# qiaozhijian/VCR-Net

Measured on NVIDIA B200. Metric: pairs/sec @1024 pts, higher is better.
Workload: dtype f16x3-split+f32acc (fp32-equivalent)

## Files before the change

### include/vcr_b200.h

```cpp
#ifndef VCR_B200_H
#define VCR_B200_H

#include <stddef.h>
#include <stdint.h>

#ifdef __cplusplus
extern "C" {
#endif

#ifndef __CUDA_RUNTIME_H__
typedef struct CUstream_st* cudaStream_t;
#endif

long long vcr_launch_count(void);
int vcr_abi_version(void);

size_t vcr_knn_workspace_bytes(int B, int N);
int vcr_knn_topk(const float* x, int B, int D, int N, int k, int token_major, int32_t* idx32,
                 int64_t* idx64, void* workspace, size_t workspace_bytes, cudaStream_t stream);

int vcr_set_knn3_direct(int on);
int vcr_set_knn_tc_tpq(int on);

size_t vcr_knn_tc_workspace_bytes(int B, int N);
int vcr_knn_topk_tc(const float* x, const void* xop, int ld, long long plane_stride, int B, int D, int N, int k,
                    int32_t* idx32, int64_t* idx64, void* workspace, size_t workspace_bytes, cudaStream_t stream);

int vcr_graph_feature(const float* xt, int B, int D, int N, int k, const int* idx, float* out,
                      cudaStream_t stream);

int vcr_fps(const float* xyz, int B, int N, int npoint, int32_t* idx32, int64_t* idx64, cudaStream_t stream);

int vcr_gemm_f32(const float* A, int lda, long long sAo, long long sAi,
                 const float* B, int ldb, long long sBo, long long sBi, int b_layout,
                 float* C, int ldc, long long sCo, long long sCi,
                 const float* bias, const float* residual, int ldr, long long sRo, long long sRi,
                 int M, int N, int K, int nb_outer, int nb_inner,
                 float alpha, int act, float slope, cudaStream_t stream);

int vcr_gemm_tc(const void* A, int lda, long long a_rows_total, int a_cols_total, long long a_plane,
                long long a_row_o, long long a_row_i, int a_col_o, int a_col_i,
                const void* B, int ldb, long long b_rows_total, int b_cols_total, long long b_plane,
                long long b_row_o, long long b_row_i, int b_col_o, int b_col_i,
                int M, int N, int K, int nb_outer, int nb_inner, int mode,
                float alpha, const float* bias, int act, float slope,
                float* C, int ldc, long long c_so, long long c_si,
                const float* R, int ldr, long long r_so, long long r_si,
                void* H, int ldh, long long h_plane, long long h_so, long long h_si, int h_split,
                void* HT, int ldt, long long t_plane, long long t_so, long long t_si,
                int out_planes, cudaStream_t stream);
int vcr_flash_attn_tc(const void* Q, int ldq, long long q_plane, const void* K, int ldk, long long k_plane,
                      const void* VT, int ldv, long long v_plane, int B, int H, int Nq, int Nk, int dk,
                      int mode, float scale, const uint8_t* keep, void* O, int ldo, long long o_plane,
                      float* lse, cudaStream_t stream);
int vcr_set_flash_warps(int nwq);
int vcr_set_gemm_pair(int on);
int vcr_gemm_quad_clusters(void);
int vcr_to_operand(const float* x, int ld, long long rows, int cols, void* out, int ldo, long long plane_stride,
                   int planes, int bf16, cudaStream_t stream);

int vcr_conv3_act(const float* xyz, const float* w, const float* bias, int B, int N, int Cout, float slope,
                  float* out, int ldo, cudaStream_t stream);
int vcr_edgeconv_dg(const float* PQ, int ldpq, const int* idx, int k, int N, long long total_pts,
                    const float* W2, const float* b2, float slope, float* x1, int ld1, float* x2, int ld2,
                    cudaStream_t stream);
int vcr_edgeconv_dg_tc(const float* PQ, int ldpq, const int* idx, int k, int N, long long total_pts,
                       const float* W2, const float* b2, float slope, int mode, float* x1, int ld1,
                       float* x2, int ld2, void* op1, void* op2, int ldop, long long op_plane, float* z,
                       cudaStream_t stream);
int vcr_gather_max(const float* P, int ldp, const float* Q, int ldq, const int* idx, int k, int N,
                   long long total_pts, int C, float slope, float* out, int ldo, void* op, int ldop,
                   long long op_plane, cudaStream_t stream);
int vcr_lpd_point_mlp(const float* xyz, const float* w1, const float* b1, const float* w2, const float* b2, int B, int N,
                      float slope, float* h1, float* h2, void* op, int ldop, long long op_plane, cudaStream_t stream);

int vcr_layernorm(const float* x, int ldx, const float* a, const float* b, float eps, long long M, int D,
                  const float* residual, int ldr, float* out, int ldo, cudaStream_t stream);
int vcr_layernorm_head(const float* x, int ldx, const float* a, const float* b, float eps, long long M, int D,
                       const float* residual, int ldr, float* out, int ldo, void* op, int ldop,
                       long long plane_stride, float* sq, cudaStream_t stream);
int vcr_softmax_rows(float* S, int ld, long long rows, int n, const uint8_t* keep, long long rows_per_batch,
                     cudaStream_t stream);
size_t vcr_colsum_workspace_bytes(int B, int n);
int vcr_colsum(const float* P, int ld, int B, long long rows_per_batch, int n, float* out, void* workspace,
               size_t workspace_bytes, cudaStream_t stream);
int vcr_layernorm_operand(const float* x, int ldx, const float* a, const float* b, float eps, long long M, int D,
                          void* out, int ldo, long long plane_stride, int planes, int bf16, cudaStream_t stream);
int vcr_row_lse(const float* S, int ld, long long rows, int n, const uint8_t* keep, long long rows_per_batch,
                float* rmax, float* rsum, cudaStream_t stream);
int vcr_softmax_operand(const float* S, int ld, long long rows, int n, const uint8_t* keep,
                        long long rows_per_batch, void* out, int ldo, long long plane_stride, int planes,
                        int bf16, cudaStream_t stream);
size_t vcr_attn_colsum_workspace_bytes(int B, int H, int Nq, int Nk);
int vcr_attn_colsum_tc(const void* Q, int ldq, long long q_plane, const void* K, int ldk, long long k_plane,
                       int B, int H, int Nq, int Nk, int dk, float scale, float* out, void* workspace,
                       size_t workspace_bytes, cudaStream_t stream);
size_t vcr_softmax_colsum_workspace_bytes(int B, long long rows_per_batch, int ld, int n);
int vcr_softmax_colsum(const float* S, int ld, int B, long long rows_per_batch, int n, float* out,
                       void* workspace, size_t workspace_bytes, cudaStream_t stream);
int vcr_colsum_softmax(const float* S, int ld, int B, long long rows_per_batch, int n, const float* rmax,
                       const float* rsum, float* out, void* workspace, size_t workspace_bytes, cudaStream_t stream);
int vcr_rowsum(const float* P, int ld, long long rows, int n, float* out, cudaStream_t stream);
int vcr_topk_select(const float* vals, int B, int n, int K, int* idx_out, uint8_t* mask_out, cudaStream_t stream);

int vcr_sqnorm_rows(const float* X, int ld, long long rows, int D, float* out, cudaStream_t stream);
int vcr_softcorr_rows(float* dot, int ld, int B, int Ns, int Nt, const float* xx, const float* yy,
                      const float* tgt, int mode, float* corr, int* best_idx, float* best_val, cudaStream_t stream);
int vcr_negdist(float* dot, int ld, int B, int Ns, int Nt, const float* xx, const float* yy, cudaStream_t stream);
int vcr_softcorr_tc(const void* S, int lds, long long s_plane, const void* T, int ldt, long long t_plane,
                    const float* xx, const float* yy, const float* tgt, int B, int Ns, int Nt, int D,
                    float* corr, cudaStream_t stream);
int vcr_softcorr_best_tc(const void* S, int lds, long long s_plane, const void* T, int ldt, long long t_plane,
                         const float* xx, const float* yy, int B, int Ns, int Nt, int D,
                         int* best_idx, float* best_val, cudaStream_t stream);
size_t vcr_select_stats_tc_workspace_bytes(int B, int Ns, int Nt);
int vcr_select_stats_tc(const void* S, int lds, long long s_plane, const void* T, int ldt, long long t_plane,
                        const float* xx, const float* yy, int B, int Ns, int Nt, int D, float* row_stat, float* col_stat,
                        void* workspace, size_t workspace_bytes, cudaStream_t stream);
size_t vcr_rowsum_colsoftmax_workspace_bytes(int B, int Nt);
int vcr_rowsum_colsoftmax(const float* pd, int ld, int B, int Ns, int Nt, float* out, void* workspace,
                          size_t workspace_bytes, cudaStream_t stream);
size_t vcr_select_stats_workspace_bytes(int B, int Ns, int Nt);
int vcr_select_stats(const float* dot, int ld, int B, int Ns, int Nt, const float* xx, const float* yy,
                     float* row_stat, float* col_stat, void* workspace, size_t workspace_bytes, cudaStream_t stream);
int vcr_gather_operand_rows(const void* in, int ld_in, long long plane_in, int B, int Nin, const int* idx, int K,
                            int C, void* out, int ld_out, long long plane_out, const float* sq_in, float* sq_out,
                            cudaStream_t stream);
int vcr_gather_rows(const float* in, int ld_in, int B, int Nin, const int* idx, int K, int C, float* out,
                    int ld_out, cudaStream_t stream);
int vcr_gather_cols(const float* in, int B, int C, int Nin, const int* idx, int K, float* out, cudaStream_t stream);
int vcr_copair_gather(const float* src, const float* tgt, int B, int Ns, int Nt, const int* keep,
                      const int* best_idx, int K, float* src_out, float* corr_out, cudaStream_t stream);

int vcr_svd_head(const float* src, const float* corr, int B, int M, float* R_ab, float* t_ab,
                 float* R_ba, float* t_ba, float* H_out, cudaStream_t stream);
int vcr_rigid_apply(const float* pc, const float* R, const float* t, int B, int N, float* out, cudaStream_t stream);
int vcr_pose_compose(const float* R_i, const float* t_i, float* R_f, float* t_f, int B, cudaStream_t stream);
int vcr_pose_inverse(const float* R, const float* t, float* R_inv, float* t_inv, int B, cudaStream_t stream);
int vcr_host_svd3(const double* H, double* U, double* S, double* V);

int vcr_transpose(const float* in, float* out, int nb, int R, int C, int ld_in, int ld_out,
                  long long stride_in, long long stride_out, cudaStream_t stream);
int vcr_add(const float* a, const float* b, float* out, long long n, cudaStream_t stream);

int vcr_make_pairs(const float* base, int P, int Nb, const int* idx_src, const int* idx_tgt, const double* pose,
                   int N, double* src64, double* tgt64, float* src, float* tgt, cudaStream_t stream);
int vcr_crop_nearest(const double* pc64, int P, int N, int keep, float* out, cudaStream_t stream);
size_t vcr_crop_nearest_workspace_bytes(int P, int N);
int vcr_crop_nearest_sort(const double* pc64, int P, int N, int keep, float* out, void* workspace, size_t workspace_bytes,
                          cudaStream_t stream);
int vcr_eval_metrics(const float* src, const float* tgt, int N, const float* srcK, const float* corrK, int M,
                     const float* R_gt, const float* t_gt, const float* R_ab, const float* t_ab,
                     const float* R_ba, const float* t_ba, int B, double* acc, cudaStream_t stream);

size_t vcr_icp_state_bytes(void);
int vcr_icp_nearest(const float* src, const float* dst, int B, int Ns, int Nt, float* corr, int* nn_idx,
                    double* err_sum, cudaStream_t stream);
int vcr_icp_advance(float* src, const float* R, const float* t, int B, int Ns, const double* err_sum,
                    float tolerance, void* state, cudaStream_t stream);

int vcr_edge_max(const float* E, int k, long long total_pts, int C, float* out, int ldo, cudaStream_t stream);

int vcr_wgrad_f32(const float* G, int ldg, const float* X, int ldx, long long M, int N, int K, float* dW,
                  int lddw, float* db, cudaStream_t stream);
int vcr_act_bwd(const float* gy, int ldg, const float* y, int ldy, long long rows, int cols, float slope,
                const int* scale_bits, float* gz, int ldz, cudaStream_t stream);
int vcr_absmax_bits(const float* x, long long n, int* bits, cudaStream_t stream);
int vcr_pow2_inverse(const int* bits, float* out, cudaStream_t stream);
int vcr_gather_max_bwd(const float* P, int ldp, const float* Q, int ldq, const int* idx, int k, int N,
                       long long total_pts, int C, float slope, const float* gout, int ldgo, float* gP,
                       int ldgp, float* gQ, int ldgq, cudaStream_t stream);
int vcr_edge_gather_act(const float* PQ, int ldpq, const int* idx, int k, int N, long long total_pts, int C,
                        float slope, float* E, cudaStream_t stream);
int vcr_edge_max_bwd(float* Z, const float* gx, int ldgx, int k, long long total_pts, int C, float slope,
                     cudaStream_t stream);
int vcr_edge_bwd_scatter(const float* E, const float* gE, const float* gx1, int ldgx, const int* idx, int k,
                         int N, long long total_pts, int C, float slope, float* gPQ, int ldg,
                         cudaStream_t stream);

#ifdef __cplusplus
}
#endif
#endif
```

### vcr_net_b200/csrc/knn.cu

```cuda
#include <atomic>
#include "tc_common.cuh"

namespace {

constexpr int TQ = 32;
constexpr int TC = 512;
constexpr int NT = 256;
constexpr int RPL = TC / 32;

template <bool TOKEN_MAJOR>
__global__ void knn_sqnorm_kernel(const float* __restrict__ x, int D, int N, float* __restrict__ xx) {
    const int b = blockIdx.y;
    const int i = blockIdx.x * blockDim.x + threadIdx.x;
    if (i >= N) return;
    const float* xb = x + (size_t)b * D * N;
    float acc = 0.f;
    for (int d = 0; d < D; ++d) {
        const float v = TOKEN_MAJOR ? xb[(size_t)i * D + d] : xb[(size_t)d * N + i];
        acc = fmaf(v, v, acc);
    }
    xx[(size_t)b * N + i] = acc;
}

__device__ __forceinline__ uint32_t okey(float v) {
    const uint32_t b = __float_as_uint(v + 0.f);
    return b ^ (uint32_t)(((int32_t)b >> 31) | 0x80000000);
}
__device__ __forceinline__ float okey_inv(uint32_t k) {
    return __uint_as_float((k & 0x80000000u) ? (k ^ 0x80000000u) : ~k);
}
struct Key { uint32_t hi, lo; };
__device__ __forceinline__ Key key_xchg(Key v, int j, bool take_max) {
    Key o;
    o.hi = __shfl_xor_sync(0xffffffffu, v.hi, j);
    o.lo = __shfl_xor_sync(0xffffffffu, v.lo, j);
    const bool gt = v.hi > o.hi || (v.hi == o.hi && v.lo > o.lo);
    return gt == take_max ? v : o;
}
__device__ __forceinline__ Key key_max(Key a, Key b) {
    return (a.hi > b.hi || (a.hi == b.hi && a.lo > b.lo)) ? a : b;
}

template <int W>
__device__ __forceinline__ void sort32_desc(Key (&v)[W], int lane) {
#pragma unroll
    for (int ks = 2; ks <= 32; ks <<= 1) {
#pragma unroll
        for (int j = ks >> 1; j > 0; j >>= 1) {
            const bool take_max = ((lane & j) == 0) == ((lane & ks) == 0);
#pragma unroll
            for (int w = 0; w < W; ++w) v[w] = key_xchg(v[w], j, take_max);
        }
    }
}
template <int W>
__device__ __forceinline__ void sort32_desc_f(float (&v)[W], int lane) {
#pragma unroll
    for (int ks = 2; ks <= 32; ks <<= 1) {
#pragma unroll
        for (int j = ks >> 1; j > 0; j >>= 1) {
            const bool take_max = ((lane & j) == 0) == ((lane & ks) == 0);
#pragma unroll
            for (int w = 0; w < W; ++w) {
                const float o = __shfl_xor_sync(0xffffffffu, v[w], j);
                v[w] = take_max ? fmaxf(v[w], o) : fminf(v[w], o);
            }
        }
    }
}
template <int W>
__device__ __forceinline__ void merge32_desc(Key (&run)[W], const Key (&add)[W], int lane) {
#pragma unroll
    for (int w = 0; w < W; ++w) {
        Key o;
        o.hi = __shfl_sync(0xffffffffu, add[w].hi, 31 - lane);
        o.lo = __shfl_sync(0xffffffffu, add[w].lo, 31 - lane);
        run[w] = key_max(run[w], o);
    }
#pragma unroll
    for (int j = 16; j > 0; j >>= 1) {
        const bool take_max = (lane & j) == 0;
#pragma unroll
        for (int w = 0; w < W; ++w) run[w] = key_xchg(run[w], j, take_max);
    }
}

template <int W, int TCN, int LDD, int CAP>
__device__ __forceinline__ bool filter_merge_t(const float* drows, const float (&tau)[W], Key (&run)[W], uint2* buf,
                                               int j0, int lane) {
    constexpr int RP = TCN / 32;
    const uint32_t lt = (1u << lane) - 1u;
    int cnt[W], off[W];
    int base = 0;
    __syncwarp();
#pragma unroll
    for (int w = 0; w < W; ++w) {
        const float* dr = drows + w * LDD + lane;
        float v[RP];
#pragma unroll
        for (int r = 0; r < RP; ++r) v[r] = dr[r * 32];
        off[w] = base;
        int n = base;
#pragma unroll
        for (int r = 0; r < RP; ++r) {
            const bool p = v[r] >= tau[w];
            const uint32_t bal = __ballot_sync(0xffffffffu, p);
            const int pos = n + __popc(bal & lt);
            if (p && pos < CAP) buf[pos] = make_uint2(~(uint32_t)(j0 + r * 32 + lane), okey(v[r]));
            n += __popc(bal);
        }
        cnt[w] = n - base;
        base = n;
    }
    __syncwarp();
    if (base > CAP) return false;
    int rounds = 0;
#pragma unroll
    for (int w = 0; w < W; ++w) rounds = max(rounds, (cnt[w] + 31) >> 5);
    for (int r = 0; r < rounds; ++r) {
        Key e[W];
#pragma unroll
        for (int w = 0; w < W; ++w) {
            const int p = r * 32 + lane;
            const uint2 t = p < cnt[w] ? buf[off[w] + p] : make_uint2(0u, 0u);
            e[w].lo = t.x; e[w].hi = t.y;
        }
        sort32_desc<W>(e, lane);
        merge32_desc<W>(run, e, lane);
    }
    return true;
}
template <int W>
__device__ __forceinline__ bool filter_merge(const float* drows, const float (&tau)[W], Key (&run)[W], uint2* buf,
                                             int j0, int lane) {
    return filter_merge_t<W, TC, TC, TC>(drows, tau, run, buf, j0, lane);
}

__device__ __forceinline__ void select_chunk(const float* dist, uint2* surv, Key (&run)[TQ / (NT / 32)], int j0, int kk,
                                             int warp, int lane, bool first) {
    constexpr int QWn = TQ / (NT / 32);
    uint2* buf = surv + (size_t)warp * TC;
    const float* drows = dist + (size_t)(warp * QWn) * TC;
    float tau[QWn];
    if (first) {
        float m[QWn];
#pragma unroll
        for (int w = 0; w < QWn; ++w) {
            const float* dr = drows + w * TC + lane;
            float mm = dr[0];
#pragma unroll
            for (int r = 1; r < RPL; ++r) mm = fmaxf(mm, dr[r * 32]);
            m[w] = mm;
        }
        sort32_desc_f<QWn>(m, lane);
#pragma unroll
        for (int w = 0; w < QWn; ++w) tau[w] = __shfl_sync(0xffffffffu, m[w], kk);
    } else {
#pragma unroll
        for (int w = 0; w < QWn; ++w) tau[w] = okey_inv(__shfl_sync(0xffffffffu, run[w].hi, kk));
    }
    if (!filter_merge<QWn>(drows, tau, run, buf, j0, lane)) {
#pragma unroll
        for (int w = 0; w < QWn; ++w) {
            float t1[1] = {tau[w]};
            Key r1[1] = {run[w]};
            filter_merge<1>(drows + w * TC, t1, r1, buf, j0, lane);
            run[w] = r1[0];
        }
    }
}

__device__ __forceinline__ void cp_async16(float* dst, const float* src, bool valid) {
    const uint32_t d = (uint32_t)__cvta_generic_to_shared(dst);
    const int sz = valid ? 16 : 0;
    asm volatile("cp.async.ca.shared.global [%0], [%1], 16, %2;\n" ::"r"(d), "l"(src), "r"(sz) : "memory");
}
__device__ __forceinline__ void cp_async_wait_all() { asm volatile("cp.async.wait_all;\n" ::: "memory"); }
__device__ __forceinline__ void cp_async_commit() { asm volatile("cp.async.commit_group;\n" ::: "memory"); }
template <int NPEND>
__device__ __forceinline__ void cp_async_wait_group() { asm volatile("cp.async.wait_group %0;\n" ::"n"(NPEND) : "memory"); }

template <int DCH, int DCP>
__device__ __forceinline__ void issue_slab(const float* __restrict__ xb, int D, int N, int j0, int q0, int d0,
                                           float* Cb, float* Qb, int tid) {
    constexpr int PPR = DCH / 4;
    constexpr int RPP = 256 / PPR;
    const int part = tid % PPR, r0 = tid / PPR;
    const bool dok = d0 + 4 * part < D;
    const float* src = xb + (size_t)(j0 + r0) * D + d0 + 4 * part;
    float* dst = Cb + r0 * DCP + 4 * part;
#pragma unroll
    for (int n = 0; n < 512 / RPP; ++n) {
        const bool ok = dok && j0 + r0 + n * RPP < N;
        cp_async16(dst + n * RPP * DCP, ok ? src + (size_t)n * RPP * D : xb, ok);
    }
    if (r0 < 32) {
        const bool ok = dok && q0 + r0 < N;
        cp_async16(Qb + r0 * DCP + 4 * part, ok ? xb + (size_t)(q0 + r0) * D + d0 + 4 * part : xb, ok);
    }
    cp_async_commit();
}

constexpr int QW = TQ / (NT / 32);
constexpr size_t SURV_BYTES = (size_t)(NT / 32) * TC * sizeof(uint2);

template <int DCH>
struct Smem {
    static constexpr int DCP = DCH == 4 ? 12 : DCH + 4;
    static constexpr size_t stage_bytes = (size_t)(TC + TQ) * DCP * sizeof(float);
    static constexpr size_t region0 = stage_bytes > SURV_BYTES ? stage_bytes : SURV_BYTES;
    static constexpr size_t total = region0 + (size_t)TC * sizeof(float) + (size_t)TQ * TC * sizeof(float);
};

template <int DCH, bool TOKEN_MAJOR>
__global__ void __launch_bounds__(NT, 2)
knn_select_kernel(const float* __restrict__ x, const float* __restrict__ xx, int D, int N, int k,
                  int32_t* __restrict__ idx32, int64_t* __restrict__ idx64, const int* __restrict__ redo) {
    if (redo != nullptr && redo[blockIdx.y * gridDim.x + blockIdx.x] == 0) return;
    using S = Smem<DCH>;
    constexpr int DCP = S::DCP;
    extern __shared__ __align__(16) unsigned char smem_raw[];
    float* Cs = reinterpret_cast<float*>(smem_raw);
    float* Qs = Cs + TC * DCP;
    uint2* surv = reinterpret_cast<uint2*>(smem_raw);
    float* xxc = reinterpret_cast<float*>(smem_raw + S::region0);
    float* dist = xxc + TC;

    const int tid = threadIdx.x, lane = tid & 31, warp = tid >> 5;
    const int qg = warp & 3, cg = warp >> 2;
    const int b = blockIdx.y, q0 = blockIdx.x * TQ;
    const float* xb = x + (size_t)b * D * N;
    const float* xxb = xx + (size_t)b * N;
    const bool vec = TOKEN_MAJOR && (D % 4 == 0) && ((reinterpret_cast<uintptr_t>(x) & 15) == 0);

    Key run[QW];
#pragma unroll
    for (int w = 0; w < QW; ++w) run[w].hi = run[w].lo = 0u;

    for (int j0 = 0; j0 < N; j0 += TC) {
        float acc[8][8];
#pragma unroll
        for (int qi = 0; qi < 8; ++qi)
#pragma unroll
            for (int ci = 0; ci < 8; ++ci) acc[qi][ci] = 0.f;

        const int nslab = (D + DCH - 1) / DCH;
        __syncthreads();
        if (vec) issue_slab<DCH, DCP>(xb, D, N, j0, q0, 0, Cs, Qs, tid);
        for (int c = tid; c < TC; c += NT) xxc[c] = (j0 + c < N) ? xxb[j0 + c] : 0.f;
        for (int si = 0; si < nslab; ++si) {
            const int d0 = si * DCH;
            const float* Cb = (vec && (si & 1)) ? dist : Cs;
            const float* Qb = Cb + TC * DCP;
            if (vec) {
                if (si + 1 < nslab) {
                    float* Cn = (si & 1) ? Cs : dist;
                    issue_slab<DCH, DCP>(xb, D, N, j0, q0, d0 + DCH, Cn, Cn + TC * DCP, tid);
                    cp_async_wait_group<1>();
                } else {
                    cp_async_wait_group<0>();
                }
            } else {
                for (int e = tid; e < (TC + TQ) * DCH; e += NT) {
                    int row, d;
                    if (TOKEN_MAJOR) { row = e / DCH; d = e - row * DCH; }
                    else if (e < TC * DCH) { d = e / TC; row = e - d * TC; }
                    else { const int e2 = e - TC * DCH; d = e2 / TQ; row = TC + e2 - d * TQ; }
                    const int g = row < TC ? j0 + row : q0 + (row - TC);
                    float v = 0.f;
                    if (g < N && d0 + d < D)
                        v = TOKEN_MAJOR ? xb[(size_t)g * D + d0 + d] : xb[(size_t)(d0 + d) * N + g];
                    Cs[row * DCP + d] = v;
                }
            }
            __syncthreads();

            const float* qrow = Qb + (qg * 8) * DCP;
            const float* crow = Cb + (cg * 256 + lane) * DCP;
            if (j0 + cg * 256 < N) {
#pragma unroll 1
            for (int d4 = 0; d4 < DCH / 4; ++d4) {
#pragma unroll
                for (int h = 0; h < 2; ++h) {
                    float4 cv[4];
#pragma unroll
                    for (int ci = 0; ci < 4; ++ci)
                        cv[ci] = *reinterpret_cast<const float4*>(crow + ((h * 4 + ci) * 32) * DCP + d4 * 4);
#pragma unroll
                    for (int qi = 0; qi < 8; ++qi) {
                        const float4 qv = *reinterpret_cast<const float4*>(qrow + qi * DCP + d4 * 4);
#pragma unroll
                        for (int ci = 0; ci < 4; ++ci) acc[qi][h * 4 + ci] = fmaf(qv.x, cv[ci].x, acc[qi][h * 4 + ci]);
#pragma unroll
                        for (int ci = 0; ci < 4; ++ci) acc[qi][h * 4 + ci] = fmaf(qv.y, cv[ci].y, acc[qi][h * 4 + ci]);
#pragma unroll
                        for (int ci = 0; ci < 4; ++ci) acc[qi][h * 4 + ci] = fmaf(qv.z, cv[ci].z, acc[qi][h * 4 + ci]);
#pragma unroll
                        for (int ci = 0; ci < 4; ++ci) acc[qi][h * 4 + ci] = fmaf(qv.w, cv[ci].w, acc[qi][h * 4 + ci]);
                    }
                }
            }
            }
            __syncthreads();
        }

        float xxq[8];
#pragma unroll
        for (int qi = 0; qi < 8; ++qi) {
            const int q = q0 + qg * 8 + qi;
            xxq[qi] = q < N ? xxb[q] : 0.f;
        }
#pragma unroll
        for (int ci = 0; ci < 8; ++ci) {
            const int c = cg * 256 + ci * 32 + lane;
            const float nxc = -xxc[c];
            const bool cvalid = j0 + c < N;
#pragma unroll
            for (int qi = 0; qi < 8; ++qi) {
                const float pd = __fsub_rn(__fsub_rn(nxc, -2.f * acc[qi][ci]), xxq[qi]);
                dist[(qg * 8 + qi) * TC + c] = cvalid ? pd : -INFINITY;
            }
        }
        __syncthreads();

        select_chunk(dist, surv, run, j0, k, warp, lane, j0 == 0);
    }

#pragma unroll
    for (int w = 0; w < QW; ++w) {
        const int q = q0 + warp * QW + w;
        if (q < N && lane >= 1 && lane <= k) {
            const int j = (int)(~run[w].lo);
            const size_t o = ((size_t)b * N + q) * k + lane - 1;
            if (idx32) idx32[o] = j;
            if (idx64) idx64[o] = (int64_t)j;
        }
    }
}

template <int DCH, bool TM>
int launch_knn(const float* x, const float* xx, int B, int D, int N, int k, int32_t* i32, int64_t* i64,
               cudaStream_t st, const int* redo = nullptr) {
    auto kern = knn_select_kernel<DCH, TM>;
    const size_t smem = Smem<DCH>::total;
    if (cudaFuncSetAttribute(kern, cudaFuncAttributeMaxDynamicSharedMemorySize, (int)smem) != cudaSuccess) return VCR_ERR_LAUNCH;
    dim3 grid(vcr_cdiv(N, TQ), B);
    kern<<<grid, NT, smem, st>>>(x, xx, D, N, k, i32, i64, redo);
    VCR_CHECK_LAUNCH();
    return VCR_OK;
}

template <int W, class F>
__device__ __forceinline__ bool filter_merge_fn(F&& get, const float (&tau)[W], Key (&run)[W], uint2* buf, int j0, int lane) {
    constexpr int RP = TC / 32;
    const uint32_t lt = (1u << lane) - 1u;
    int cnt[W], off[W];
    int base = 0;
    __syncwarp();
#pragma unroll
    for (int w = 0; w < W; ++w) {
        off[w] = base;
        int n = base;
#pragma unroll
        for (int r = 0; r < RP; ++r) {
            const float v = get(w, r);
            const bool p = v >= tau[w];
            const uint32_t bal = __ballot_sync(0xffffffffu, p);
            const int pos = n + __popc(bal & lt);
            if (p && pos < TC) buf[pos] = make_uint2(~(uint32_t)(j0 + r * 32 + lane), okey(v));
            n += __popc(bal);
        }
        cnt[w] = n - base;
        base = n;
    }
    __syncwarp();
    if (base > TC) return false;
    int rounds = 0;
#pragma unroll
    for (int w = 0; w < W; ++w) rounds = max(rounds, (cnt[w] + 31) >> 5);
    for (int r = 0; r < rounds; ++r) {
        Key e[W];
#pragma unroll
        for (int w = 0; w < W; ++w) {
            const int p = r * 32 + lane;
            const uint2 t = p < cnt[w] ? buf[off[w] + p] : make_uint2(0u, 0u);
            e[w].lo = t.x; e[w].hi = t.y;
        }
        sort32_desc<W>(e, lane);
        merge32_desc<W>(run, e, lane);
    }
    return true;
}

constexpr int QW3 = 2;
constexpr int TQ3 = QW3 * (NT / 32);
template <bool TOKEN_MAJOR>
__global__ void __launch_bounds__(NT, 4)
knn3_kernel(const float* __restrict__ x, const float* __restrict__ xx, int N, int k,
            int32_t* __restrict__ idx32, int64_t* __restrict__ idx64) {
    __shared__ float cs[4][TC];
    __shared__ uint2 surv[NT / 32][TC];
    const int tid = threadIdx.x, lane = tid & 31, warp = tid >> 5;
    const int b = blockIdx.y, q0 = blockIdx.x * TQ3;
    const float* xb = x + (size_t)b * 3 * N;
    const float* xxb = xx + (size_t)b * N;

    float qx[QW3], qy[QW3], qz[QW3], xxq[QW3];
#pragma unroll
    for (int w = 0; w < QW3; ++w) {
        const int q = min(q0 + warp * QW3 + w, N - 1);
        qx[w] = TOKEN_MAJOR ? xb[(size_t)q * 3 + 0] : xb[q];
        qy[w] = TOKEN_MAJOR ? xb[(size_t)q * 3 + 1] : xb[(size_t)N + q];
        qz[w] = TOKEN_MAJOR ? xb[(size_t)q * 3 + 2] : xb[2 * (size_t)N + q];
        xxq[w] = xxb[q];
    }
    Key run[QW3];
#pragma unroll
    for (int w = 0; w < QW3; ++w) run[w].hi = run[w].lo = 0u;
    uint2* buf = surv[warp];

    for (int j0 = 0; j0 < N; j0 += TC) {
        __syncthreads();
        for (int c = tid; c < TC; c += NT) {
            const int g = j0 + c;
            const bool ok = g < N;
            cs[0][c] = ok ? (TOKEN_MAJOR ? xb[(size_t)g * 3 + 0] : xb[g]) : 0.f;
            cs[1][c] = ok ? (TOKEN_MAJOR ? xb[(size_t)g * 3 + 1] : xb[(size_t)N + g]) : 0.f;
            cs[2][c] = ok ? (TOKEN_MAJOR ? xb[(size_t)g * 3 + 2] : xb[2 * (size_t)N + g]) : 0.f;
            cs[3][c] = ok ? xxb[g] : 0.f;
        }
        __syncthreads();
        auto pd = [&](int w, int r) -> float {
            const int c = r * 32 + lane;
            const float acc = fmaf(qz[w], cs[2][c], fmaf(qy[w], cs[1][c], fmaf(qx[w], cs[0][c], 0.f)));
            const float v = __fsub_rn(__fsub_rn(-cs[3][c], -2.f * acc), xxq[w]);
            return j0 + c < N ? v : -INFINITY;
        };
        float tau[QW3];
        if (j0 == 0) {
            float m[QW3];
#pragma unroll
            for (int w = 0; w < QW3; ++w) {
                float mm = pd(w, 0);
#pragma unroll
                for (int r = 1; r < RPL; ++r) mm = fmaxf(mm, pd(w, r));
                m[w] = mm;
            }
            sort32_desc_f<QW3>(m, lane);
#pragma unroll
            for (int w = 0; w < QW3; ++w) tau[w] = __shfl_sync(0xffffffffu, m[w], k);
        } else {
#pragma unroll
            for (int w = 0; w < QW3; ++w) tau[w] = okey_inv(__shfl_sync(0xffffffffu, run[w].hi, k));
        }
        if (!filter_merge_fn<QW3>(pd, tau, run, buf, j0, lane)) {
#pragma unroll
            for (int w = 0; w < QW3; ++w) {
                float t1[1] = {tau[w]};
                Key r1[1] = {run[w]};
                filter_merge_fn<1>([&](int, int r) { return pd(w, r); }, t1, r1, buf, j0, lane);
                run[w] = r1[0];
            }
        }
    }
#pragma unroll
    for (int w = 0; w < QW3; ++w) {
        const int q = q0 + warp * QW3 + w;
        if (q < N && lane >= 1 && lane <= k) {
            const int j = (int)(~run[w].lo);
            const size_t o = ((size_t)b * N + q) * k + lane - 1;
            if (idx32) idx32[o] = j;
            if (idx64) idx64[o] = (int64_t)j;
        }
    }
}

constexpr int T2M = 128;
constexpr int T2TILES = TC / T2M;
constexpr int T2NT = NT + 32;
constexpr int T2CTILE = T2M * 128;
constexpr int T2QTILE = TQ * 128;

struct KnnTcParams {
    const float* x;
    const float* xx;
    const uint32_t* xxmax;
    int* redo;
    int* nflag;
    int D, N, k, ksel, KB;
    int32_t* idx32;
    int64_t* idx64;
};

__host__ __device__ constexpr size_t knn_tc_stage_bytes(int KB) {
    return (size_t)KB * 2 * T2CTILE > SURV_BYTES ? (size_t)KB * 2 * T2CTILE : SURV_BYTES;
}
__host__ __device__ constexpr size_t knn_tc_smem_bytes(int KB) {
    return (size_t)KB * 2 * T2QTILE + knn_tc_stage_bytes(KB) + (size_t)TQ * TC * 4 + TQ * 4 + 64 + 1024;
}

__global__ void knn_sqnorm_max_kernel(const float* __restrict__ x, int D, int N, float* __restrict__ xx,
                                      uint32_t* __restrict__ xxmax) {
    const int b = blockIdx.y;
    const int i = blockIdx.x * blockDim.x + threadIdx.x;
    uint32_t bits = 0u;
    if (i < N) {
        const float* r = x + ((size_t)b * N + i) * D;
        float acc = 0.f;
        for (int d = 0; d < D; ++d) acc = fmaf(r[d], r[d], acc);
        xx[(size_t)b * N + i] = acc;
        bits = __float_as_uint(acc);
    }
    bits = __reduce_max_sync(0xffffffffu, bits);
    if ((threadIdx.x & 31) == 0 && bits) atomicMax(xxmax + b, bits);
}

__global__ void __launch_bounds__(T2NT, 2)
knn_tc_kernel(const __grid_constant__ CUtensorMap tmC, const __grid_constant__ CUtensorMap tmQ, const KnnTcParams p) {
    extern __shared__ uint8_t smem_raw[];
    uint8_t* smem = smem_raw + ((1024u - (tc::smem_u32(smem_raw) & 1023u)) & 1023u);
    const int KB = p.KB, N = p.N, D = p.D, k = p.k, ksel = p.ksel;
    const int qbytes = KB * 2 * T2QTILE, cbytes = KB * 2 * T2CTILE;
    uint8_t* q_s = smem;
    uint8_t* c_s = smem + qbytes;
    uint2* surv = reinterpret_cast<uint2*>(c_s);
    float* dist = reinterpret_cast<float*>(c_s + knn_tc_stage_bytes(KB));
    float* xxq_s = dist + TQ * TC;
    uint64_t* bars = reinterpret_cast<uint64_t*>(xxq_s + TQ);
    uint64_t* q_full = bars + 0;
    uint64_t* c_full = bars + 1;
    uint64_t* mma_bar = bars + 2;
    uint64_t* chunk_ready = bars + 3;
    uint64_t* stage_free = bars + 4;
    uint32_t* tmem_slot = reinterpret_cast<uint32_t*>(bars + 5);

    const int tid = threadIdx.x, warp = tid >> 5, lane = tid & 31;
    const int b = blockIdx.y, q0 = blockIdx.x * TQ;
    const float* xxb = p.xx + (size_t)b * N;
    const int nch = (N + TC - 1) / TC;

    if (warp == NT / 32 && lane == 0) {
        tc::tma_prefetch_desc(&tmC); tc::tma_prefetch_desc(&tmQ);
        tc::mbar_init(q_full, 1); tc::mbar_init(c_full, 1); tc::mbar_init(mma_bar, 1);
        tc::mbar_init(chunk_ready, 1); tc::mbar_init(stage_free, NT / 32);
        tc::fence_barrier_init();
    }
    if (warp == 0) { tc::tmem_alloc(tmem_slot, 256); tc::tmem_relinquish(); }
    if (tid < TQ) xxq_s[tid] = q0 + tid < N ? xxb[q0 + tid] : 0.f;
    tc::tc_fence_before();
    __syncthreads();
    tc::tc_fence_after();
    const uint32_t tmem_base = *tmem_slot;

    const float xm = __uint_as_float(p.xxmax[b]);
    const bool cloud_ok = xm >= 9.5367431640625e-07f && xm <= 1073741824.f;
    if (!cloud_ok) {
        if (tid == 0) {
            p.redo[b * gridDim.x + blockIdx.x] = 1;
            atomicAdd(p.nflag, min(TQ, N - q0));
        }
    } else if (warp == NT / 32) {
        if (tc::elect_one()) {
            constexpr uint32_t idesc = tc::umma_idesc(T2M, TQ, 0);
            const int row0 = b * N;
            tc::mbar_expect_tx(q_full, qbytes);
            for (int kb = 0; kb < KB; ++kb)
                for (int pl = 0; pl < 2; ++pl)
                    tc::tma_load_3d(q_s + (kb * 2 + pl) * T2QTILE, &tmQ, q_full, kb * 64, row0 + q0, pl);
            tc::mbar_wait(q_full, 0);
            const uint32_t q_addr = tc::smem_u32(q_s), c_addr = tc::smem_u32(c_s);
            uint32_t g = 0;
            for (int c = 0; c < nch; ++c) {
                if (c > 0) { tc::mbar_wait(stage_free, (c - 1) & 1); tc::tc_fence_after(); }
                for (int t = 0; t < T2TILES; ++t, ++g) {
                    const int cand0 = c * TC + t * T2M;
                    if (cand0 < N) {
                        tc::mbar_expect_tx(c_full, cbytes);
                        for (int kb = 0; kb < KB; ++kb)
                            for (int pl = 0; pl < 2; ++pl)
                                tc::tma_load_3d(c_s + (kb * 2 + pl) * T2CTILE, &tmC, c_full, kb * 64, row0 + cand0, pl);
                        tc::mbar_wait(c_full, g & 1);
                        tc::tc_fence_after();
                        const uint32_t d0 = tmem_base + t * TQ, d1 = tmem_base + T2TILES * TQ + t * TQ;
                        for (int kb = 0; kb < KB; ++kb) {
                            const uint64_t c_hi = tc::umma_desc_k_sw128(c_addr + (kb * 2) * T2CTILE);
                            const uint64_t c_lo = tc::umma_desc_k_sw128(c_addr + (kb * 2 + 1) * T2CTILE);
                            const uint64_t q_hi = tc::umma_desc_k_sw128(q_addr + (kb * 2) * T2QTILE);
                            const uint64_t q_lo = tc::umma_desc_k_sw128(q_addr + (kb * 2 + 1) * T2QTILE);
#pragma unroll
                            for (int kk = 0; kk < 4; ++kk) {
                                const uint32_t acc = (kb | kk) != 0;
                                const uint64_t adv = (uint64_t)(kk * 2);
                                tc::umma_f16(d0, c_hi + adv, q_hi + adv, idesc, acc);
                                tc::umma_f16(d1, c_hi + adv, q_lo + adv, idesc, acc);
                                tc::umma_f16(d1, c_lo + adv, q_hi + adv, idesc, 1);
                            }
                        }
                        tc::umma_commit(mma_bar);
                        tc::mbar_wait(mma_bar, g & 1);
                    } else {
                        tc::mbar_arrive(c_full);
                        tc::mbar_arrive(mma_bar);
                    }
                }
                tc::umma_commit(chunk_ready);
            }
        }
    } else {
        const int qq = warp & 3, th = warp >> 2;
        Key run[QW];
#pragma unroll
        for (int w = 0; w < QW; ++w) run[w].hi = run[w].lo = 0u;

        for (int c = 0; c < nch; ++c) {
            const int j0 = c * TC;
            tc::mbar_wait(chunk_ready, c & 1);
            tc::tc_fence_after();
#pragma unroll
            for (int tt = 0; tt < T2TILES / 2; ++tt) {
                const int t = th * (T2TILES / 2) + tt;
                const int cl = t * T2M + qq * 32 + lane;
                const int j = j0 + cl;
                float* dcol = dist + cl;
                if (j0 + t * T2M < N) {
                    const uint32_t ta = tmem_base + ((uint32_t)(qq * 32) << 16) + t * TQ;
                    const bool cvalid = j < N;
                    const float nxc = cvalid ? -xxb[j] : 0.f;
#pragma unroll
                    for (int h = 0; h < 2; ++h) {
                        uint32_t r0[16], r1[16];
                        tc::tmem_ld_32x16(ta + h * 16, r0);
                        tc::tmem_ld_32x16(ta + T2TILES * TQ + h * 16, r1);
                        tc::tmem_ld_wait();
#pragma unroll
                        for (int q = 0; q < 16; ++q) {
                            const float dot = fmaf(__uint_as_float(r1[q]), 1.f / 2048.f, __uint_as_float(r0[q]));
                            const float pd = __fsub_rn(__fsub_rn(nxc, -2.f * dot), xxq_s[h * 16 + q]);
                            dcol[(h * 16 + q) * TC] = cvalid ? pd : -INFINITY;
                        }
                    }
                } else {
#pragma unroll
                    for (int q = 0; q < TQ; ++q) dcol[q * TC] = -INFINITY;
                }
            }
            tc::tc_fence_before();
            asm volatile("bar.sync 1, %0;" ::"n"(NT) : "memory");
            select_chunk(dist, surv, run, j0, ksel, warp, lane, c == 0);
            tc::fence_proxy_async();
            __syncwarp();
            if (lane == 0) tc::mbar_arrive(stage_free);
        }

        const bool vec = (D % 4 == 0) && ((reinterpret_cast<uintptr_t>(p.x) & 15) == 0);
        bool all_safe = true;
#pragma unroll
        for (int qi = 0; qi < QW; ++qi) {
            const int q = q0 + warp * QW + qi;
            if (q >= N) continue;
            const Key a = run[qi];
            const uint32_t thr_hi = __shfl_sync(0xffffffffu, a.hi, ksel);
            const int j = (int)(~a.lo);
            const bool valid = j >= 0 && j < N;
            const float xxq = xxq_s[warp * QW + qi];
            Key e[1];
            e[0].hi = 0u; e[0].lo = 0u;
            if (valid) {
                const float* xq = p.x + ((size_t)b * N + q) * D;
                const float* xj = p.x + ((size_t)b * N + j) * D;
                float acc = 0.f;
                if (vec) {
                    for (int d = 0; d < D; d += 4) {
                        const float4 qv = __ldg(reinterpret_cast<const float4*>(xq + d));
                        const float4 cv = __ldg(reinterpret_cast<const float4*>(xj + d));
                        acc = fmaf(qv.x, cv.x, acc); acc = fmaf(qv.y, cv.y, acc);
                        acc = fmaf(qv.z, cv.z, acc); acc = fmaf(qv.w, cv.w, acc);
                    }
                } else {
                    for (int d = 0; d < D; ++d) acc = fmaf(__ldg(xq + d), __ldg(xj + d), acc);
                }
                const float pd = __fsub_rn(__fsub_rn(-xxb[j], -2.f * acc), xxq);
                e[0].hi = okey(pd); e[0].lo = a.lo;
            }
            sort32_desc<1>(e, lane);
            const uint32_t ek_hi = __shfl_sync(0xffffffffu, e[0].hi, k);
            const float eps = 6.103515625e-05f * sqrtf(xxq * xm) + 9.5367431640625e-07f * xm;
            const bool safe = ek_hi != 0u && (thr_hi == 0u || okey_inv(ek_hi) > okey_inv(thr_hi) + eps);
            if (safe) {
                if (lane >= 1 && lane <= k) {
                    const int jn = (int)(~e[0].lo);
                    const size_t o = ((size_t)b * N + q) * k + lane - 1;
                    if (p.idx32) p.idx32[o] = jn;
                    if (p.idx64) p.idx64[o] = (int64_t)jn;
                }
            } else {
                all_safe = false;
                if (lane == 0) atomicAdd(p.nflag, 1);
            }
        }
        if (!all_safe && lane == 0) p.redo[b * gridDim.x + blockIdx.x] = 1;
    }
    tc::tc_fence_before();
    __syncthreads();
    if (warp == 0) tc::tmem_dealloc(tmem_base, 256);
}

#include "knn_tpq.cuh"

}

VCR_API size_t vcr_knn_workspace_bytes(int B, int N) { return (size_t)B * N * sizeof(float); }

static std::atomic<int> g_vcr_knn3_direct{1};
static std::atomic<int> g_vcr_knn_tc_tpq{2};

VCR_API int vcr_set_knn3_direct(int on) {
    return g_vcr_knn3_direct.exchange(on ? 1 : 0);
}

VCR_API int vcr_set_knn_tc_tpq(int on) {
    return g_vcr_knn_tc_tpq.exchange(on < 0 ? 0 : (on > 2 ? 2 : on));
}

VCR_API int vcr_knn_topk(const float* x, int B, int D, int N, int k, int token_major, int32_t* idx32,
                         int64_t* idx64, void* workspace, size_t workspace_bytes, cudaStream_t stream) {
    VCR_REQUIRE(x && (idx32 || idx64) && B > 0 && N > 0 && k >= 1);
    if (N < k + 1) return VCR_ERR_INVALID;
    if (!workspace || workspace_bytes < vcr_knn_workspace_bytes(B, N)) return VCR_ERR_WORKSPACE;
    float* xx = reinterpret_cast<float*>(workspace);
    dim3 g(vcr_cdiv(N, 256), B);
    if (token_major) knn_sqnorm_kernel<true><<<g, 256, 0, stream>>>(x, D, N, xx);
    else knn_sqnorm_kernel<false><<<g, 256, 0, stream>>>(x, D, N, xx);
    VCR_CHECK_LAUNCH();
    if (k > 31) return VCR_ERR_UNSUPPORTED;
    const int route3 = g_vcr_knn3_direct.load(std::memory_order_relaxed);
    if (D == 3 && route3 != 0) {
        dim3 grid(vcr_cdiv(N, TQ3), B);
        if (token_major) knn3_kernel<true><<<grid, NT, 0, stream>>>(x, xx, N, k, idx32, idx64);
        else knn3_kernel<false><<<grid, NT, 0, stream>>>(x, xx, N, k, idx32, idx64);
        VCR_CHECK_LAUNCH();
        return VCR_OK;
    }
    if (D <= 4)
        return token_major ? launch_knn<4, true>(x, xx, B, D, N, k, idx32, idx64, stream)
                           : launch_knn<4, false>(x, xx, B, D, N, k, idx32, idx64, stream);
    return token_major ? launch_knn<16, true>(x, xx, B, D, N, k, idx32, idx64, stream)
                       : launch_knn<16, false>(x, xx, B, D, N, k, idx32, idx64, stream);
}

VCR_API size_t vcr_knn_tc_workspace_bytes(int B, int N) {
    return ((size_t)B * N + (size_t)B + (size_t)B * ((N + 31) / 32) + 1) * 4;
}

VCR_API int vcr_knn_topk_tc(const float* x, const void* xop, int ld, long long plane_stride, int B, int D, int N, int k,
                            int32_t* idx32, int64_t* idx64, void* workspace, size_t workspace_bytes,
                            cudaStream_t stream) {
    VCR_REQUIRE(x && xop && (idx32 || idx64) && B > 0 && N > 0 && k >= 1);
    if (N < k + 1) return VCR_ERR_INVALID;
    if (D < 16 || D > 128 || k > 30 || (long long)B * N > 0x7fffffffLL || B > 65535) return VCR_ERR_UNSUPPORTED;
    if (!workspace || workspace_bytes < vcr_knn_tc_workspace_bytes(B, N)) return VCR_ERR_WORKSPACE;
    const int nq32 = (N + 31) / 32;
    float* xx = reinterpret_cast<float*>(workspace);
    uint32_t* xxmax = reinterpret_cast<uint32_t*>(xx + (size_t)B * N);
    int* redo = reinterpret_cast<int*>(xxmax + B);
    int* nflag = redo + (size_t)B * nq32;
    if (cudaMemsetAsync(xxmax, 0, ((size_t)B + (size_t)B * nq32 + 1) * 4, stream) != cudaSuccess) return VCR_ERR_LAUNCH;
    dim3 g(vcr_cdiv(N, 256), B);
    knn_sqnorm_max_kernel<<<g, 256, 0, stream>>>(x, D, N, xx, xxmax);
    VCR_CHECK_LAUNCH();
    CUtensorMap tmC, tmQ;
    const int tpq = g_vcr_knn_tc_tpq.load(std::memory_order_relaxed);
    if (tpq == 1 || (tpq == 2 && N >= 8192)) {
        int rc = vcr_make_operand_tmap(&tmC, xop, D, (long long)B * N, ld, plane_stride, 2, TC2);
        if (rc != VCR_OK) return rc;
        rc = vcr_make_operand_tmap(&tmQ, xop, D, (long long)B * N, ld, plane_stride, 2, TQ2);
        if (rc != VCR_OK) return rc;
        KnnTcParams p;
        p.x = x; p.xx = xx; p.xxmax = xxmax; p.redo = redo; p.nflag = nflag;
        p.D = D; p.N = N; p.k = k; p.ksel = k + 8 < 31 ? k + 8 : 31; p.KB = (D + 63) / 64;
        p.idx32 = idx32; p.idx64 = idx64;
        const size_t smem = knn_tc2_smem_bytes(p.KB);
        if (cudaFuncSetAttribute(knn_tc2_kernel, cudaFuncAttributeMaxDynamicSharedMemorySize, (int)smem) != cudaSuccess)
            return VCR_ERR_LAUNCH;
        knn_tc2_kernel<<<dim3(vcr_cdiv(N, TQ2), B), T2_THREADS, smem, stream>>>(tmC, tmQ, p);
        VCR_CHECK_LAUNCH();
        return launch_knn<16, true>(x, xx, B, D, N, k, idx32, idx64, stream, redo);
    }
    int rc = vcr_make_operand_tmap(&tmC, xop, D, (long long)B * N, ld, plane_stride, 2, T2M);
    if (rc != VCR_OK) return rc;
    rc = vcr_make_operand_tmap(&tmQ, xop, D, (long long)B * N, ld, plane_stride, 2, TQ);
    if (rc != VCR_OK) return rc;
    KnnTcParams p;
    p.x = x; p.xx = xx; p.xxmax = xxmax; p.redo = redo; p.nflag = nflag;
    p.D = D; p.N = N; p.k = k; p.ksel = k + 8 < 31 ? k + 8 : 31; p.KB = (D + 63) / 64;
    p.idx32 = idx32; p.idx64 = idx64;
    const size_t smem = knn_tc_smem_bytes(p.KB);
    if (cudaFuncSetAttribute(knn_tc_kernel, cudaFuncAttributeMaxDynamicSharedMemorySize, (int)smem) != cudaSuccess)
        return VCR_ERR_LAUNCH;
    knn_tc_kernel<<<dim3(nq32, B), T2NT, smem, stream>>>(tmC, tmQ, p);
    VCR_CHECK_LAUNCH();
    return launch_knn<16, true>(x, xx, B, D, N, k, idx32, idx64, stream, redo);
}
```

Before: 3739.

## Add whole-row KNN kernels with threshold-based top-k selection for small N

Adds row kernels for N up to 1024 that hold every candidate distance for a query row in registers or shared memory. A warp-level threshold estimate keeps only candidates above the k-th value, compacts those survivors, then sorts and merges them, replacing the tiled streaming filter-merge. Distances come from a cp.async double-buffered FP32 GEMM for token-major D divisible by 4, and from a direct kernel for D=3. Costs are heavier shared-memory use (one block per SM in the general kernel) and new routing that depends on alignment and layout.

```diff
diff --git a/include/vcr_b200.h b/include/vcr_b200.h
--- a/include/vcr_b200.h
+++ b/include/vcr_b200.h
@@ -20,6 +20,7 @@
                  int64_t* idx64, void* workspace, size_t workspace_bytes, cudaStream_t stream);
 
 int vcr_set_knn3_direct(int on);
+int vcr_set_knn_row(int on);
 int vcr_set_knn_tc_tpq(int on);
 
 size_t vcr_knn_tc_workspace_bytes(int B, int N);
diff --git a/vcr_net_b200/csrc/knn.cu b/vcr_net_b200/csrc/knn.cu
--- a/vcr_net_b200/csrc/knn.cu
+++ b/vcr_net_b200/csrc/knn.cu
@@ -475,6 +475,302 @@
     }
 }
 
+constexpr int QR = 2;
+constexpr int TQR = QR * (NT / 32);
+
+template <int RP, class F>
+__device__ __forceinline__ void select_row(const float (&v)[QR][RP], F&& value, uint16_t* buf, int kk, int lane,
+                                           Key (&out)[QR]) {
+    float m[2 * QR];
+#pragma unroll
+    for (int w = 0; w < QR; ++w) {
+        float a = v[w][0], b = v[w][RP / 2];
+#pragma unroll
+        for (int r = 1; r < RP / 2; ++r) { a = fmaxf(a, v[w][r]); b = fmaxf(b, v[w][RP / 2 + r]); }
+        m[2 * w] = a; m[2 * w + 1] = b;
+    }
+    sort32_desc_f<2 * QR>(m, lane);
+    float tau[QR];
+#pragma unroll
+    for (int w = 0; w < QR; ++w) tau[w] = fmaxf(m[2 * w], __shfl_sync(0xffffffffu, m[2 * w + 1], 31 - lane));
+#pragma unroll
+    for (int j = 16; j > 0; j >>= 1) {
+        const bool take_max = (lane & j) == 0;
+#pragma unroll
+        for (int w = 0; w < QR; ++w) {
+            const float o = __shfl_xor_sync(0xffffffffu, tau[w], j);
+            tau[w] = take_max ? fmaxf(tau[w], o) : fminf(tau[w], o);
+        }
+    }
+    int cnt[QR], incl[QR];
+#pragma unroll
+    for (int w = 0; w < QR; ++w) {
+        tau[w] = __shfl_sync(0xffffffffu, tau[w], kk);
+        int c = 0;
+#pragma unroll
+        for (int r = 0; r < RP; ++r) c += v[w][r] >= tau[w];
+        cnt[w] = incl[w] = c;
+    }
+#pragma unroll
+    for (int d = 1; d < 32; d <<= 1) {
+#pragma unroll
+        for (int w = 0; w < QR; ++w) {
+            const int t = __shfl_up_sync(0xffffffffu, incl[w], d);
+            if (lane >= d) incl[w] += t;
+        }
+    }
+    int total[QR], rounds = 0;
+    __syncwarp();
+#pragma unroll
+    for (int w = 0; w < QR; ++w) {
+        total[w] = __shfl_sync(0xffffffffu, incl[w], 31);
+        rounds = max(rounds, (total[w] + 31) >> 5);
+        uint16_t* b = buf + w * RP * 32 + (incl[w] - cnt[w]);
+#pragma unroll
+        for (int r = 0; r < RP; ++r)
+            if (v[w][r] >= tau[w]) *b++ = (uint16_t)(r * 32 + lane);
+    }
+    __syncwarp();
+    for (int rd = 0; rd < rounds; ++rd) {
+        Key e[QR];
+#pragma unroll
+        for (int w = 0; w < QR; ++w) {
+            const int p = rd * 32 + lane;
+            e[w].hi = e[w].lo = 0u;
+            if (p < total[w]) {
+                const int j = buf[w * RP * 32 + p];
+                e[w].hi = okey(value(w, j)); e[w].lo = ~(uint32_t)j;
+            }
+        }
+        sort32_desc<QR>(e, lane);
+        if (rd == 0) {
+#pragma unroll
+            for (int w = 0; w < QR; ++w) out[w] = e[w];
+        } else {
+            merge32_desc<QR>(out, e, lane);
+        }
+    }
+}
+
+__device__ __forceinline__ void store_row(const Key& run, int b, int q, int N, int k, int lane, int32_t* idx32,
+                                          int64_t* idx64) {
+    if (q < N && lane >= 1 && lane <= k) {
+        const int j = (int)(~run.lo);
+        const size_t o = ((size_t)b * N + q) * k + lane - 1;
+        if (idx32) idx32[o] = j;
+        if (idx64) idx64[o] = (int64_t)j;
+    }
+}
+
+constexpr int RNT = 512;
+constexpr int RTQ = QR * (RNT / 32);
+constexpr int RDCH = 8, RDCP = 12;
+template <int RP>
+struct RowSmem {
+    static constexpr int NC = RP * 32;
+    static constexpr size_t slab_floats = (size_t)(NC + RTQ) * RDCP;
+    static constexpr size_t slabs = 2 * slab_floats * sizeof(float);
+    static constexpr size_t tile = (size_t)RTQ * NC * 4 + (size_t)(RNT / 32) * QR * NC * 2;
+    static constexpr size_t region0 = slabs > tile ? slabs : tile;
+    static constexpr size_t total = region0 + (size_t)NC * sizeof(float);
+};
+
+template <int RP>
+__device__ __forceinline__ void issue_row_slab(const float* __restrict__ xb, int D, int N, int q0, int d0, float* Cb,
+                                               float* Qb, int tid) {
+    constexpr int NC = RP * 32;
+    const int part = tid & 1, r0 = tid >> 1;
+    const bool dok = d0 + 4 * part < D;
+#pragma unroll
+    for (int n = 0; n < NC / 256; ++n) {
+        const int row = r0 + n * 256;
+        const bool ok = dok && row < N;
+        cp_async16(Cb + row * RDCP + 4 * part, ok ? xb + (size_t)row * D + d0 + 4 * part : xb, ok);
+    }
+    if (r0 < RTQ) {
+        const bool ok = dok && q0 + r0 < N;
+        cp_async16(Qb + r0 * RDCP + 4 * part, ok ? xb + (size_t)(q0 + r0) * D + d0 + 4 * part : xb, ok);
+    }
+    cp_async_commit();
+}
+
+template <int RP>
+__global__ void __launch_bounds__(RNT, 1)
+knn_row_kernel(const float* __restrict__ x, const float* __restrict__ xx, int D, int N, int k,
+               int32_t* __restrict__ idx32, int64_t* __restrict__ idx64) {
+    using S = RowSmem<RP>;
+    constexpr int NC = S::NC;
+    extern __shared__ __align__(16) unsigned char smem_raw[];
+    float* slab0 = reinterpret_cast<float*>(smem_raw);
+    float* dist = slab0;
+    uint16_t* surv = reinterpret_cast<uint16_t*>(dist + RTQ * NC);
+    float* xxc = reinterpret_cast<float*>(smem_raw + S::region0);
+
+    const int tid = threadIdx.x, lane = tid & 31, warp = tid >> 5;
+    const int qg = warp & 3, cg = warp >> 2;
+    const int b = blockIdx.y, q0 = blockIdx.x * RTQ;
+    const float* xb = x + (size_t)b * D * N;
+    const float* xxb = xx + (size_t)b * N;
+
+    float acc[8][8];
+#pragma unroll
+    for (int qi = 0; qi < 8; ++qi)
+#pragma unroll
+        for (int ci = 0; ci < 8; ++ci) acc[qi][ci] = 0.f;
+
+    const int nslab = (D + RDCH - 1) / RDCH;
+    issue_row_slab<RP>(xb, D, N, q0, 0, slab0, slab0 + NC * RDCP, tid);
+    for (int c = tid; c < NC; c += RNT) xxc[c] = c < N ? xxb[c] : 0.f;
+    for (int si = 0; si < nslab; ++si) {
+        const float* Cb = slab0 + (si & 1) * S::slab_floats;
+        const float* Qb = Cb + NC * RDCP;
+        if (si + 1 < nslab) {
+            float* Cn = slab0 + ((si + 1) & 1) * S::slab_floats;
+            issue_row_slab<RP>(xb, D, N, q0, (si + 1) * RDCH, Cn, Cn + NC * RDCP, tid);
+            cp_async_wait_group<1>();
+        } else {
+            cp_async_wait_group<0>();
+        }
+        __syncthreads();
+        const float* qrow = Qb + (qg * 8) * RDCP;
+        const float* crow = Cb + (cg * 256 + lane) * RDCP;
+        if (cg * 256 < NC) {
+#pragma unroll 1
+            for (int d4 = 0; d4 < RDCH / 4; ++d4) {
+#pragma unroll
+                for (int h = 0; h < 2; ++h) {
+                    float4 cv[4];
+#pragma unroll
+                    for (int ci = 0; ci < 4; ++ci)
+                        cv[ci] = *reinterpret_cast<const float4*>(crow + ((h * 4 + ci) * 32) * RDCP + d4 * 4);
+#pragma unroll
+                    for (int qi = 0; qi < 8; ++qi) {
+                        const float4 qv = *reinterpret_cast<const float4*>(qrow + qi * RDCP + d4 * 4);
+#pragma unroll
+                        for (int ci = 0; ci < 4; ++ci) acc[qi][h * 4 + ci] = fmaf(qv.x, cv[ci].x, acc[qi][h * 4 + ci]);
+#pragma unroll
+                        for (int ci = 0; ci < 4; ++ci) acc[qi][h * 4 + ci] = fmaf(qv.y, cv[ci].y, acc[qi][h * 4 + ci]);
+#pragma unroll
+                        for (int ci = 0; ci < 4; ++ci) acc[qi][h * 4 + ci] = fmaf(qv.z, cv[ci].z, acc[qi][h * 4 + ci]);
+#pragma unroll
+                        for (int ci = 0; ci < 4; ++ci) acc[qi][h * 4 + ci] = fmaf(qv.w, cv[ci].w, acc[qi][h * 4 + ci]);
+                    }
+                }
+            }
+        }
+        __syncthreads();
+    }
+
+    if (cg * 256 < NC) {
+        float xxq[8];
+#pragma unroll
+        for (int qi = 0; qi < 8; ++qi) {
+            const int q = q0 + qg * 8 + qi;
+            xxq[qi] = q < N ? xxb[q] : 0.f;
+        }
+#pragma unroll
+        for (int ci = 0; ci < 8; ++ci) {
+            const int c = cg * 256 + ci * 32 + lane;
+            const float nxc = -xxc[c];
+            const bool cvalid = c < N;
+#pragma unroll
+            for (int qi = 0; qi < 8; ++qi) {
+                const float pd = __fsub_rn(__fsub_rn(nxc, -2.f * acc[qi][ci]), xxq[qi]);
+                dist[(qg * 8 + qi) * NC + c] = cvalid ? pd : -INFINITY;
+            }
+        }
+    }
+    __syncthreads();
+
+    const float* drow = dist + (warp * QR) * NC;
+    float v[QR][RP];
+#pragma unroll
+    for (int w = 0; w < QR; ++w)
+#pragma unroll
+        for (int r = 0; r < RP; ++r) v[w][r] = drow[w * NC + r * 32 + lane];
+    Key run[QR];
+    select_row<RP>(v, [&](int w, int j) { return drow[w * NC + j]; }, surv + warp * QR * NC, k, lane, run);
+#pragma unroll
+    for (int w = 0; w < QR; ++w) store_row(run[w], b, q0 + warp * QR + w, N, k, lane, idx32, idx64);
+}
+
+template <int RP>
+int launch_knn_row(const float* x, const float* xx, int B, int D, int N, int k, int32_t* i32, int64_t* i64,
+                   cudaStream_t st) {
+    auto kern = knn_row_kernel<RP>;
+    const size_t smem = RowSmem<RP>::total;
+    if (cudaFuncSetAttribute(kern, cudaFuncAttributeMaxDynamicSharedMemorySize, (int)smem) != cudaSuccess) return VCR_ERR_LAUNCH;
+    kern<<<dim3(vcr_cdiv(N, RTQ), B), RNT, smem, st>>>(x, xx, D, N, k, i32, i64);
+    VCR_CHECK_LAUNCH();
+    return VCR_OK;
+}
+
+__device__ __forceinline__ float pd3(float qx, float qy, float qz, float xxq, float cx, float cy, float cz, float cxx) {
+    const float acc = fmaf(qz, cz, fmaf(qy, cy, fmaf(qx, cx, 0.f)));
+    return __fsub_rn(__fsub_rn(-cxx, -2.f * acc), xxq);
+}
+
+template <int RP, bool TOKEN_MAJOR>
+__global__ void __launch_bounds__(NT, 2)
+knn3_row_kernel(const float* __restrict__ x, const float* __restrict__ xx, int N, int k,
+                int32_t* __restrict__ idx32, int64_t* __restrict__ idx64) {
+    constexpr int NC = RP * 32;
+    __shared__ float cs[4][NC];
+    __shared__ uint16_t surv[NT / 32][QR * NC];
+    const int tid = threadIdx.x, lane = tid & 31, warp = tid >> 5;
+    const int b = blockIdx.y, q0 = blockIdx.x * TQR;
+    const float* xb = x + (size_t)b * 3 * N;
+    const float* xxb = xx + (size_t)b * N;
+
+    for (int c = tid; c < NC; c += NT) {
+        const bool ok = c < N;
+        cs[0][c] = ok ? (TOKEN_MAJOR ? xb[(size_t)c * 3 + 0] : xb[c]) : 0.f;
+        cs[1][c] = ok ? (TOKEN_MAJOR ? xb[(size_t)c * 3 + 1] : xb[(size_t)N + c]) : 0.f;
+        cs[2][c] = ok ? (TOKEN_MAJOR ? xb[(size_t)c * 3 + 2] : xb[2 * (size_t)N + c]) : 0.f;
+        cs[3][c] = ok ? xxb[c] : 0.f;
+    }
+    float qx[QR], qy[QR], qz[QR], xxq[QR];
+#pragma unroll
+    for (int w = 0; w < QR; ++w) {
+        const int q = min(q0 + warp * QR + w, N - 1);
+        qx[w] = TOKEN_MAJOR ? xb[(size_t)q * 3 + 0] : xb[q];
+        qy[w] = TOKEN_MAJOR ? xb[(size_t)q * 3 + 1] : xb[(size_t)N + q];
+        qz[w] = TOKEN_MAJOR ? xb[(size_t)q * 3 + 2] : xb[2 * (size_t)N + q];
+        xxq[w] = xxb[q];
+    }
+    __syncthreads();
+
+    float v[QR][RP];
+#pragma unroll
+    for (int r = 0; r < RP; ++r) {
+        const int c = r * 32 + lane;
+        const float cx = cs[0][c], cy = cs[1][c], cz = cs[2][c], cxx = cs[3][c];
+#pragma unroll
+        for (int w = 0; w < QR; ++w) {
+            const float pd = pd3(qx[w], qy[w], qz[w], xxq[w], cx, cy, cz, cxx);
+            v[w][r] = c < N ? pd : -INFINITY;
+        }
+    }
+    auto value = [&](int w, int j) -> float {
+        const float pd = pd3(qx[w], qy[w], qz[w], xxq[w], cs[0][j], cs[1][j], cs[2][j], cs[3][j]);
+        return j < N ? pd : -INFINITY;
+    };
+    Key run[QR];
+    select_row<RP>(v, value, surv[warp], k, lane, run);
+#pragma unroll
+    for (int w = 0; w < QR; ++w) store_row(run[w], b, q0 + warp * QR + w, N, k, lane, idx32, idx64);
+}
+
+template <int RP>
+int launch_knn3_row(const float* x, const float* xx, int B, int N, int k, int tm, int32_t* i32, int64_t* i64,
+                    cudaStream_t st) {
+    const dim3 grid(vcr_cdiv(N, TQR), B);
+    if (tm) knn3_row_kernel<RP, true><<<grid, NT, 0, st>>>(x, xx, N, k, i32, i64);
+    else knn3_row_kernel<RP, false><<<grid, NT, 0, st>>>(x, xx, N, k, i32, i64);
+    VCR_CHECK_LAUNCH();
+    return VCR_OK;
+}
+
 constexpr int T2M = 128;
 constexpr int T2TILES = TC / T2M;
 constexpr int T2NT = NT + 32;
@@ -713,6 +1009,11 @@
 
 static std::atomic<int> g_vcr_knn3_direct{1};
 static std::atomic<int> g_vcr_knn_tc_tpq{2};
+static std::atomic<int> g_vcr_knn_row{1};
+
+VCR_API int vcr_set_knn_row(int on) {
+    return g_vcr_knn_row.exchange(on ? 1 : 0);
+}
 
 VCR_API int vcr_set_knn3_direct(int on) {
     return g_vcr_knn3_direct.exchange(on ? 1 : 0);
@@ -734,6 +1035,23 @@
     VCR_CHECK_LAUNCH();
     if (k > 31) return VCR_ERR_UNSUPPORTED;
     const int route3 = g_vcr_knn3_direct.load(std::memory_order_relaxed);
+    const int rp = N <= 1024 && g_vcr_knn_row.load(std::memory_order_relaxed) ? 8 * vcr_cdiv(N, 256) : 0;
+    if (D == 3 && route3 != 0 && rp) {
+        switch (rp) {
+            case 8: return launch_knn3_row<8>(x, xx, B, N, k, token_major, idx32, idx64, stream);
+            case 16: return launch_knn3_row<16>(x, xx, B, N, k, token_major, idx32, idx64, stream);
+            case 24: return launch_knn3_row<24>(x, xx, B, N, k, token_major, idx32, idx64, stream);
+            default: return launch_knn3_row<32>(x, xx, B, N, k, token_major, idx32, idx64, stream);
+        }
+    }
+    if (D >= 4 && D % 4 == 0 && token_major && (reinterpret_cast<uintptr_t>(x) & 15) == 0 && rp) {
+        switch (rp) {
+            case 8: return launch_knn_row<8>(x, xx, B, D, N, k, idx32, idx64, stream);
+            case 16: return launch_knn_row<16>(x, xx, B, D, N, k, idx32, idx64, stream);
+            case 24: return launch_knn_row<24>(x, xx, B, D, N, k, idx32, idx64, stream);
+            default: return launch_knn_row<32>(x, xx, B, D, N, k, idx32, idx64, stream);
+        }
+    }
     if (D == 3 && route3 != 0) {
         dim3 grid(vcr_cdiv(N, TQ3), B);
         if (token_major) knn3_kernel<true><<<grid, NT, 0, stream>>>(x, xx, N, k, idx32, idx64);
```

Result: faster. 3801 (median of 6 runs) (+1.6%).
